# ComputationalPhysiology/oasisx

Hardware: AMD Instinct MI355X
Metric: time-steps/sec, 3D Taylor-Green 128^3 P2-P1 (with pressure-CG SpMV GB/s in roofline) (higher is better)
Workload: dtype f64

## Files before the change

### include/oasisx_hip.h

```cpp
#ifndef OASISX_HIP_H
#define OASISX_HIP_H

#include <stddef.h>
#include <stdint.h>

#ifdef __cplusplus
extern "C" {
#endif

#define OX_KV 2
#define OX_ROW_BLOCK_WAVES 8
#define OX_ROW_BLOCK_LDS (134 * 1024)
#define OX_SLICE 64

#define OX_CONVERGED_RTOL 2
#define OX_CONVERGED_ATOL 3
#define OX_CONVERGED_ITS 4
#define OX_DIVERGED_ITS (-3)
#define OX_DIVERGED_DTOL (-4)
#define OX_DIVERGED_BREAKDOWN (-5)
#define OX_DIVERGED_NANORINF (-9)

#define OX_KSP_CG 1
#define OX_KSP_BCGS 2
// ... 1 lines not shown
#define OX_KSP_BCGS_MERGED 4

#define OX_KSP_CG_MERGED 5

typedef struct {
  int64_t n_rows;
  int64_t n_cols;
  int32_t n_slices;
  int32_t n_dict;
  const int64_t *slice_ptr;
  const int32_t *cols;
  double *vals;
  const uint16_t *cols16;
  const int32_t *cbase;
  const uint8_t *vcode;
  const double *vdict;
  const int32_t *ib_slices;
  int32_t n_interior;
  int32_t n_wb_interior;
  const int64_t *ps_ptr;
  const uint32_t *ps_code;
  const int32_t *ps_base;
  const int32_t *wb_slices;
  const uint16_t *wb_waves;
  const int64_t *wb_ptr;
  const int32_t *wlist;
  const int64_t *wt_ptr;
  const uint16_t *wcode;
  const uint8_t *wvcode;
  int32_t n_wblocks;
  int32_t w_max;
  int32_t levels;
  int32_t w_cap;
} ox_sell;
#define OX_SPMV_LEVELS(mask) (32 | ((mask) & 31))

typedef struct {
  int32_t gdim;
  int32_t reserved;
  int64_t n_cells;
  const double *geom;
} ox_cells;

typedef struct {
  int32_t n_slices;
  int32_t nd;
  const int64_t *adj_ptr;
  const int32_t *adj_cell;
  const uint8_t *adj_loc;
} ox_adj;

typedef struct ox_dist ox_dist;

typedef struct {
  int32_t reason[4];
  int32_t its[4];
  double rnorm[4];
  double bnorm[4];
  int32_t resumed[4];
} ox_ksp_result;

typedef struct ox_mesh ox_mesh;
typedef struct ox_space ox_space;
typedef struct ox_rect ox_rect;

typedef struct {
  int32_t gdim, tile_bits;
  int64_t n_vertices, n_cells;
// ... 65 lines not shown
                       int on_device, const double *lo, const double *span, int lattice, int tile_bits,
                       int64_t n_cells_whole, ox_mesh **out);
int ox_space_create_part(const ox_mesh *mesh, int degree, int window, const int32_t *owner, int64_t n_initial, int rank,
                         int64_t n_dofs_whole, ox_space **out);
int ox_space_view(const ox_space *space, ox_space_info *view);
int ox_space_windows(ox_space *space, ox_window_info *view);
int ox_space_windows_split(ox_space *space, int split_entries, ox_window_info *view);
int ox_space_destroy(ox_space *space);
int ox_rect_create(const ox_space *rows, const ox_space *cols, ox_rect **out);
int ox_rect_view(const ox_rect *rect, ox_rect_info *view);
int ox_rect_destroy(ox_rect *rect);
int ox_value_dictionary(const double *vals, int64_t n_slots, int ncomp, void *codes, double *dict, int *n_dict,
                        void *stream);
int ox_pair_stream_size(const ox_sell *A, const int32_t *row_len, int64_t *ps_ptr, int64_t *n_codes, void *stream);
int ox_window_retile(const ox_sell *A, const int64_t *wt_ptr, const void *src, int elem_bytes, void *dst, void *stream);
int ox_pair_stream_fill(const ox_sell *A, const int32_t *row_len, int64_t *ps_ptr, uint32_t *ps_code,
                        int32_t *ps_base, int64_t *n_wide, void *stream);
int ox_malloc(size_t bytes, void **out);
int ox_free(void *p);
int ox_memset(void *p, int value, size_t bytes, void *stream);
int ox_synchronize(void *stream);

int ox_version(void);
const char *ox_last_error(void);
int ox_sell_kv(void);
int ox_device_info(int *n_cu, char *name, int name_len);

int ox_spmv(const ox_sell *A, const double *x, double *y, int ncomp, const ox_dist *dist,
            void *stream);

int ox_sell_compress_cols(const ox_sell *A, uint16_t *cols16, int32_t *cbase, int64_t *n_compressed,
                          void *stream);

int ox_spmv_multi(int v2s, int gdim, const ox_sell *A, const double *x, const double *base, double scale,
                  double *y, const ox_dist *dist, void *stream);
int ox_assemble_rect(int family, int row_degree, int col_degree, const ox_cells *cells, const ox_adj *adj,
                     const uint8_t *adj_pos, int pw, const ox_sell *A, void *stream);

int ox_axpby(int64_t n, double a, const double *x, double b, const double *y, double *z,
             void *stream);
int ox_dot(int64_t n_rows, int ncomp, const double *x, const double *y, double *out_host,
           const ox_dist *dist, void *stream);

int ox_set_bc(double *b, const int32_t *dofs, const double *g, int64_t n, int ncomp, int comp,
              void *stream);

int ox_scatter_add(double *b, const int32_t *rows, const double *y, int64_t n, int ncomp, int comp,
                   double scale, void *stream);

int ox_zero_rows(const ox_sell *A, const int32_t *rows, int64_t n, double diag, void *stream);
int ox_zero_rows_au(const ox_sell *A, const int32_t *rows, int64_t n, double diag, double *au,
                    const double *u1, int ncomp, void *stream);
int ox_zero_rows_cols(const ox_sell *A, const uint8_t *is_bc, double diag, void *stream);

int ox_assemble_matrix(int kind, int degree, const ox_cells *cells, const int32_t *cell_dofs,
                       const ox_adj *adj, const uint8_t *adj_pos, int pw, const ox_sell *A,
                       int n_bins, const int64_t *bin_ptr_host, const int32_t *bin_slices,
                       const int32_t *bin_width_host, void *stream);
int ox_assemble_weights(int degree, const ox_cells *cells, const ox_adj *adj, int64_t n_rows,
                        double *w, void *stream);
int ox_assemble_load_vector(const ox_cells *cells, const ox_adj *adj, int64_t n_rows, int n_d, int n_q,
                            const double *wphi, const double *fq, double *b, void *stream);

int ox_assemble_first(int degree, const ox_cells *cells, const int32_t *cell_dofs,
                      const ox_adj *adj, const uint8_t *adj_pos, int pw, const ox_sell *A,
                      const ox_sell *M, const ox_sell *K, const double *uab,
// ... 190 lines not shown
```

### oasisx_amd/_lib.py

```python
from __future__ import annotations

import ctypes as C
import os

_HERE = os.path.dirname(os.path.abspath(__file__))
LIB_PATH = os.environ.get("OX_LIB_PATH") or os.path.join(_HERE, "liboasisx_hip.so")

KSP_CG, KSP_BCGS, KSP_CG_SINGLE, KSP_BCGS_MERGED, KSP_CG_MERGED = 1, 2, 3, 4, 5
KSP_CG_MG = 6
MG_MAX_DEGREE = 8
ROW_BLOCK_WAVES, ROW_BLOCK_LDS = 8, 134 * 1024
CONVERGED_RTOL, CONVERGED_ATOL, CONVERGED_ITS = 2, 3, 4
DIVERGED_ITS, DIVERGED_DTOL, DIVERGED_BREAKDOWN, DIVERGED_NANORINF = -3, -4, -5, -9


class OasisxHipError(RuntimeError):
    pass


class ox_sell(C.Structure):
    _fields_ = [
        ("n_rows", C.c_int64),
        ("n_cols", C.c_int64),
        ("n_slices", C.c_int32),
        ("n_dict", C.c_int32),
        ("slice_ptr", C.c_void_p),
        ("cols", C.c_void_p),
        ("vals", C.c_void_p),
        ("cols16", C.c_void_p),
        ("cbase", C.c_void_p),
        ("vcode", C.c_void_p),
        ("vdict", C.c_void_p),
        ("ib_slices", C.c_void_p),
        ("n_interior", C.c_int32),
        ("n_wb_interior", C.c_int32),
        ("ps_ptr", C.c_void_p),
        ("ps_code", C.c_void_p),
        ("ps_base", C.c_void_p),
        ("wb_slices", C.c_void_p),
        ("wb_waves", C.c_void_p),
        ("wb_ptr", C.c_void_p),
        ("wlist", C.c_void_p),
        ("wt_ptr", C.c_void_p),
        ("wcode", C.c_void_p),
        ("wvcode", C.c_void_p),
        ("n_wblocks", C.c_int32),
        ("w_max", C.c_int32),
        ("levels", C.c_int32),
        ("w_cap", C.c_int32),
    ]


class ox_window_info(C.Structure):
    _fields_ = [
        ("n_wblocks", C.c_int32),
        ("w_max", C.c_int32),
        ("n_list", C.c_int64),
        ("n_tiles", C.c_int64),
        ("n_over_16bit", C.c_int64),
        ("wb_slices", C.c_void_p),
        ("wb_waves", C.c_void_p),
        ("wb_ptr", C.c_void_p),
        ("wlist", C.c_void_p),
        ("wt_ptr", C.c_void_p),
        ("wcode", C.c_void_p),
    ]


class ox_cells(C.Structure):
    _fields_ = [
        ("gdim", C.c_int32),
        ("reserved", C.c_int32),
        ("n_cells", C.c_int64),
        ("geom", C.c_void_p),
    ]


class ox_adj(C.Structure):
    _fields_ = [
        ("n_slices", C.c_int32),
        ("nd", C.c_int32),
        ("adj_ptr", C.c_void_p),
# ... 113 lines not shown
_P = C.c_void_p
_I = C.c_int
_L = C.c_int64
_D = C.c_double

SIGNATURES = {
    "ox_version": (_I, []),
    "ox_last_error": (C.c_char_p, []),
    "ox_sell_kv": (_I, []),
    "ox_device_info": (_I, [C.POINTER(_I), C.c_char_p, _I]),
    "ox_mesh_create": (_I, [_P, _L, _P, _L, _I, _I, _I, C.POINTER(_P)]),
    "ox_mesh_view": (_I, [_P, C.POINTER(ox_mesh_info)]),
    "ox_mesh_destroy": (_I, [_P]),
    "ox_space_create": (_I, [_P, _I, _I, C.POINTER(_P)]),
    "ox_space_create_ordered": (_I, [_P, _I, _I, _I, C.POINTER(_P)]),
    "ox_mesh_create_sub": (_I, [_P, _L, _P, _L, _I, _I, C.POINTER(_D), C.POINTER(_D), _I, _I, _L, C.POINTER(_P)]),
    "ox_space_create_part": (_I, [_P, _I, _I, _P, _L, _I, _L, C.POINTER(_P)]),
    "ox_space_view": (_I, [_P, C.POINTER(ox_space_info)]),
    "ox_space_windows": (_I, [_P, C.POINTER(ox_window_info)]),
    "ox_space_windows_split": (_I, [_P, _I, C.POINTER(ox_window_info)]),
    "ox_space_destroy": (_I, [_P]),
    "ox_rect_create": (_I, [_P, _P, C.POINTER(_P)]),
    "ox_rect_view": (_I, [_P, C.POINTER(ox_rect_info)]),
    "ox_rect_destroy": (_I, [_P]),
    "ox_value_dictionary": (_I, [_P, _L, _I, _P, _P, C.POINTER(_I), _P]),
    "ox_pair_stream_size": (_I, [C.POINTER(ox_sell), _P, _P, C.POINTER(_L), _P]),
    "ox_pair_stream_fill": (_I, [C.POINTER(ox_sell), _P, _P, _P, _P, C.POINTER(_L), _P]),
    "ox_malloc": (_I, [C.c_size_t, C.POINTER(_P)]),
    "ox_free": (_I, [_P]),
    "ox_memset": (_I, [_P, _I, C.c_size_t, _P]),
    "ox_synchronize": (_I, [_P]),
    "ox_spmv": (_I, [C.POINTER(ox_sell), _P, _P, _I, _P, _P]),
    "ox_sell_compress_cols": (_I, [C.POINTER(ox_sell), _P, _P, C.POINTER(_L), _P]),
    "ox_spmv_multi": (_I, [_I, _I, C.POINTER(ox_sell), _P, _P, _D, _P, _P, _P]),
    "ox_assemble_rect": (_I, [_I, _I, _I, C.POINTER(ox_cells), C.POINTER(ox_adj), _P, _I, C.POINTER(ox_sell), _P]),
    "ox_axpby": (_I, [_L, _D, _P, _D, _P, _P, _P]),
    "ox_dot": (_I, [_L, _I, _P, _P, C.POINTER(_D), _P, _P]),
    "ox_set_bc": (_I, [_P, _P, _P, _L, _I, _I, _P]),
    "ox_scatter_add": (_I, [_P, _P, _P, _L, _I, _I, _D, _P]),
    "ox_zero_rows": (_I, [C.POINTER(ox_sell), _P, _L, _D, _P]),
    "ox_zero_rows_au": (_I, [C.POINTER(ox_sell), _P, _L, _D, _P, _P, _I, _P]),
    "ox_zero_rows_cols": (_I, [C.POINTER(ox_sell), _P, _D, _P]),
    "ox_assemble_matrix": (_I, [_I, _I, C.POINTER(ox_cells), _P, C.POINTER(ox_adj), _P, _I,
                                C.POINTER(ox_sell), _I, C.POINTER(_L), _P, C.POINTER(C.c_int32), _P]),
    "ox_assemble_weights": (_I, [_I, C.POINTER(ox_cells), C.POINTER(ox_adj), _L, _P, _P]),
    "ox_assemble_load_vector": (_I, [C.POINTER(ox_cells), C.POINTER(ox_adj), _L, _I, _I, _P, _P, _P, _P]),
    "ox_assemble_first": (_I, [_I, C.POINTER(ox_cells), _P, C.POINTER(ox_adj), _P, _I,
                               C.POINTER(ox_sell), C.POINTER(ox_sell), C.POINTER(ox_sell), _P, _P, _P, _P, _D,
                               _D, _I, C.POINTER(_L), _P, C.POINTER(C.c_int32), _P]),
    "ox_assemble_first_au": (_I, [_I, C.POINTER(ox_cells), _P, C.POINTER(ox_adj), _P, _I,
                                  C.POINTER(ox_sell), C.POINTER(ox_sell), C.POINTER(ox_sell), _P, _P, _P, _P, _D,
                                  _D, _I, C.POINTER(_L), _P, C.POINTER(C.c_int32), _P, _P]),
    "ox_assemble_matrix_blocks": (_I, [_I, _I, C.POINTER(ox_cells), _P, C.POINTER(ox_adj), _P, _I, C.POINTER(ox_sell), _I, _P,
                                       _L, _P]),
    "ox_assemble_first_blocks": (_I, [_I, C.POINTER(ox_cells), _P, C.POINTER(ox_adj), _P, _I,
                                      C.POINTER(ox_sell), C.POINTER(ox_sell), C.POINTER(ox_sell), _P, _P, _P, _P, _D,
                                      _D, _I, _P, _L, _P, _P]),
    "ox_eddy_viscosity": (_I, [_I, _I, C.POINTER(ox_cells), _P, _P, _D, _P, _P]),
    "ox_assemble_first_au_nut": (_I, [_I, C.POINTER(ox_cells), _P, C.POINTER(ox_adj), _P, _I,
                                      C.POINTER(ox_sell), C.POINTER(ox_sell), C.POINTER(ox_sell), _P, _P, _P, _P, _D,
                                      _D, _I, C.POINTER(_L), _P, C.POINTER(C.c_int32), _P, _P, _P]),
    "ox_assemble_first_blocks_nut": (_I, [_I, C.POINTER(ox_cells), _P, C.POINTER(ox_adj), _P, _I,
                                          C.POINTER(ox_sell), C.POINTER(ox_sell), C.POINTER(ox_sell), _P, _P, _P, _P, _D,
                                          _D, _I, _P, _L, _P, _P, _P]),
    "ox_viscosity_law": (_I, [_I, _I, C.POINTER(ox_cells), _P, _P, C.POINTER(_D), _I, _P, _P]),
    "ox_assemble_stress_transpose": (_I, [_I, C.POINTER(ox_cells), _P, C.POINTER(ox_adj), _L, _P, _P, _D, _P, _P]),
# ... 117 lines not shown
```

### oasisx_amd/csrc/ox_spmv.hip

```cpp
#include "ox_common.h"
#include "ox_kernels.h"
#include <stdlib.h>
#include <type_traits>

thread_local char ox_err_buf[512] = "";

extern "C" int ox_version(void) { return 100; }
extern "C" const char *ox_last_error(void) { return ox_err_buf; }
extern "C" int ox_sell_kv(void) { return OX_KV; }

extern "C" int ox_device_info(int *n_cu, char *name, int name_len) {
  int dev = 0;
  OX_HIP(hipGetDevice(&dev));
  hipDeviceProp_t p;
  OX_HIP(hipGetDeviceProperties(&p, dev));
  if (n_cu) *n_cu = p.multiProcessorCount;
  if (name && name_len > 0) {
    strncpy(name, p.gcnArchName, name_len - 1);
    name[name_len - 1] = 0;
  }
  return 0;
}

template <int NC, int EPI, int VAR>
// ... 34 lines not shown
    const int64_t base = A.slice_ptr[slice];
    const int npair = (int)((A.slice_ptr[slice + 1] - base) >> 7);
    const double2 *__restrict__ vp = reinterpret_cast<const double2 *>(A.vals + base) + lane;
    typedef double v2d __attribute__((ext_vector_type(2)));
    typedef int v2i __attribute__((ext_vector_type(2)));
    typedef unsigned short v2h __attribute__((ext_vector_type(2)));
    const unsigned short *__restrict__ vcp =
        (VAR & 4) ? reinterpret_cast<const unsigned short *>(A.vcode + base) + lane : nullptr;
    auto load_vals = [&](int k) {
      double2 v;
      if (VAR & 4) {
        const unsigned cc = __builtin_nontemporal_load(vcp + (size_t)k * 64);
        v.x = dict[cc & 0xff];
        v.y = dict[cc >> 8];
      } else if (VAR & 1) {
        const v2d vv = __builtin_nontemporal_load(reinterpret_cast<const v2d *>(vp + (size_t)k * 64));
        v.x = vv.x;
        v.y = vv.y;
      } else {
        v = vp[(size_t)k * 64];
      }
      return v;
    };
    auto mac = [&](double2 v, int c0, int c1) {
      const double *x0 = x + (size_t)c0 * NC;
      const double *x1 = x + (size_t)c1 * NC;
#pragma unroll
      for (int cc = 0; cc < NC; ++cc) acc[cc] = fma(v.x, x0[cc], acc[cc]);
#pragma unroll
      for (int cc = 0; cc < NC; ++cc) acc[cc] = fma(v.y, x1[cc], acc[cc]);
    };
    const int2 *__restrict__ cb =
        (VAR & 2) ? reinterpret_cast<const int2 *>(A.cbase) + (base >> 7) : nullptr;
    if ((VAR & 2) && cb[0].x >= 0) {
      const v2h *__restrict__ hp = reinterpret_cast<const v2h *>(A.cols16 + base) + lane;
#pragma unroll 4
      for (int k = 0; k < npair; ++k) {
        const double2 v = load_vals(k);
        const v2h d = __builtin_nontemporal_load(hp + (size_t)k * 64);
        const int2 b = cb[k];
        const int dx = d.x, dy = d.y;
        mac(v, ((dx & 0x8000) ? b.y : b.x) + (dx & 0x7fff), ((dy & 0x8000) ? b.y : b.x) + (dy & 0x7fff));
      }
    } else {
      const int2 *__restrict__ cp = reinterpret_cast<const int2 *>(A.cols + base) + lane;
#pragma unroll 4
      for (int k = 0; k < npair; ++k) {
        const double2 v = load_vals(k);
        int2 c;
        if (VAR & 1) {
          const v2i ci = __builtin_nontemporal_load(reinterpret_cast<const v2i *>(cp + (size_t)k * 64));
          c.x = ci.x;
          c.y = ci.y;
        } else {
          c = cp[(size_t)k * 64];
        }
        mac(v, c.x, c.y);
      }
    }
    if (row < A.n_rows) {
      if (EPI == OX_EPI_BCGS_V || EPI == OX_EPI_BCGS_T || EPI == OX_EPI_BCGS_T5) {
        const double d = dinv[row];
#pragma unroll
        for (int c = 0; c < NC; ++c) acc[c] *= d;
      }
#pragma unroll
      for (int c = 0; c < NC; ++c) y[row * NC + c] = acc[c];
// ... 373 lines not shown
            const double dd = ED.code ? ED.dict[ED.code[row]] : dinv[row];
            s[c] = fma(x[row * NC + c], acc[c], s[c]);
            s[NC + c] = fma(acc[c], dd * acc[c], s[NC + c]);
          }
        }
      }
    }
  }
  if (EPI != OX_EPI_NONE) {
    ox_block_sum_256<NV>(s, red);
    if (threadIdx.x == 0) {
#pragma unroll
      for (int i = 0; i < NV; ++i) partial[(size_t)blockIdx.x * NV + i] = s[i];
    }
  }
}

#include <mutex>
static const int *ox_zero_flag(hipStream_t st) {
  static std::mutex mu;
  static int *z[16] = {};
  int dev = 0;
  if (hipGetDevice(&dev) != hipSuccess || dev < 0 || dev >= 16) return nullptr;
  std::lock_guard<std::mutex> lock(mu);
  if (!z[dev]) {
    int *p = nullptr;
    if (hipMalloc(&p, 64) != hipSuccess) return nullptr;
    if (hipMemsetAsync(p, 0, 64, st) != hipSuccess || hipStreamSynchronize(st) != hipSuccess) return nullptr;
    z[dev] = p;
  }
  return z[dev];
}

#define OX_SPMV_DEFAULT_VARIANT 31
static inline int spmv_levels(const ox_sell *A) { return (A->levels & 32) ? (A->levels & 31) : OX_SPMV_DEFAULT_VARIANT; }

static int spmv_window_cap(const ox_sell *A, int ncomp, const int32_t *list) {
  if (list && !(A->ib_slices && (list == A->ib_slices || list == A->ib_slices + A->n_interior))) return 0;
  if (!(spmv_levels(A) & 16) || !A->wcode || !A->wt_ptr || !A->wlist || !A->wb_ptr || !A->wb_slices ||
      !A->wb_waves || A->n_wblocks <= 0 || ncomp < 1 || ncomp > 3)
    return 0;
  const int dflt = ncomp == 1 ? 6144 : (ncomp == 2 ? 3072 : 2176);
  const int cap = A->w_cap > 0 ? A->w_cap : dflt;
  return A->w_max < cap ? A->w_max : cap;
}
static inline int spmv_window_grid_n(int nblocks) { return (nblocks + 7) & ~7; }
static inline void spmv_window_range(const ox_sell *A, const int32_t *list, int n_list, int *first, int *count) {
  if (!list) *first = 0, *count = A->n_wblocks;
  else if (list == A->ib_slices && n_list == A->n_interior) *first = 0, *count = A->n_wb_interior;
  else *first = A->n_wb_interior, *count = A->n_wblocks - A->n_wb_interior;
}

static thread_local OxEpiDinv g_epi_dinv{nullptr, nullptr};
void ox_spmv_set_epilogue_dinv(const uint8_t *code, const double *dict) { g_epi_dinv = OxEpiDinv{code, dict}; }

static int spmv_launch_list(const ox_sell *A, const double *x, double *y, int ncomp, int epi,
                            const double *dinv, const double *aux, double *partial, const int *done,
                            hipStream_t st, const int32_t *list, int n_list) {
  const int nblk = list ? ox_spmv_blocks_n(n_list) : ox_spmv_blocks(A);
  if (nblk == 0) return 0;
  const int lv = spmv_levels(A);
  int var = (A->cols16 && A->cbase) ? (lv & 7) : (lv & 1);
  const bool pairs = (lv & 8) && A->ps_ptr && A->ps_code && A->ps_base;
  if ((var & 6) != 6 || !A->vcode || !A->vdict || A->n_dict < 1 || A->n_dict > 256) var &= 3;
  else var = 7;
  const int w_cap = pairs ? 0 : spmv_window_cap(A, ncomp, list);
  if (w_cap > 0) {
    const bool codes = var == 7 && A->wvcode;
    int wb0 = 0, wbn = 0;
    spmv_window_range(A, list, n_list, &wb0, &wbn);
    if (wbn == 0) return 0;
    const int wgrid = spmv_window_grid_n(wbn);
    const size_t lds = (size_t)w_cap * ncomp * sizeof(double);
#define OX_WIN_CASE(NC, E)                                                                                          \
  if (ncomp == NC && epi == E) {                                                                                    \
    auto go = [&](auto kern) -> int {                                                                               \
      if (lds > 48 * 1024)                                                                                          \
        OX_HIP(hipFuncSetAttribute(reinterpret_cast<const void *>(kern), hipFuncAttributeMaxDynamicSharedMemorySize, \
                                   (int)lds));                                                                      \
      if (ox_prof_on) ox_prof_start(OX_TAG_SPMV(NC, E), st, A->n_rows);                                             \
      hipLaunchKernelGGL(kern, dim3(wgrid), dim3(256), lds, st, *A, x, y, dinv, aux, partial, done, w_cap, g_epi_dinv, wb0, wbn); \
      if (ox_prof_on) ox_prof_stop(st);                                                                             \
      OX_LAUNCH_CHECK();                                                                                            \
      return 0;                                                                                                     \
    };                                                                                                              \
    return codes ? go(k_spmv_win<NC, E, 5>) : go(k_spmv_win<NC, E, 1>);                                             \
  }
#define OX_WIN_NC(NC)                                                                                   \
  OX_WIN_CASE(NC, OX_EPI_NONE) OX_WIN_CASE(NC, OX_EPI_DOT) OX_WIN_CASE(NC, OX_EPI_BCGS_V) OX_WIN_CASE(NC, OX_EPI_BCGS_T) \
  OX_WIN_CASE(NC, OX_EPI_BCGS_T5) OX_WIN_CASE(NC, OX_EPI_CG_M2)
    OX_WIN_NC(1) OX_WIN_NC(2) OX_WIN_NC(3)
#undef OX_WIN_NC
#undef OX_WIN_CASE
  }
#define OX_SPMV_LAUNCH(NC, E, V)                                                                   \
  hipLaunchKernelGGL((k_spmv<NC, E, V>), dim3(nblk), dim3(256), 0, st, *A, x, y, dinv, aux, partial, done, list, n_list, g_epi_dinv)
#define OX_SPMV_CASE(NC, E)                                                                     \
  if (ncomp == NC && epi == E) {                                                                \
    if (ox_prof_on) ox_prof_start(OX_TAG_SPMV(NC, E), st, A->n_rows);                                      \
    if (var == 7 && pairs) {                                                                    \
      const int *dz = done ? done : ox_zero_flag(st);                                             \
      if (!dz) OX_FAIL("ox_spmv: no device flag");                                              \
      hipLaunchKernelGGL((k_spmv_ps<NC, E>), dim3(nblk), dim3(256), 0, st, *A, x, y, dinv, aux, partial, dz, list, n_list, g_epi_dinv); \
    } else if (var == 7) OX_SPMV_LAUNCH(NC, E, 7);                                              \
    else if (var == 3) OX_SPMV_LAUNCH(NC, E, 3);                                                \
    else if (var == 2) OX_SPMV_LAUNCH(NC, E, 2);                                                \
    else if (var == 1) OX_SPMV_LAUNCH(NC, E, 1);                                                \
    else OX_SPMV_LAUNCH(NC, E, 0);                                                              \
    if (ox_prof_on) ox_prof_stop(st);                                                           \
    OX_LAUNCH_CHECK();                                                                          \
    return 0;                                                                                   \
  }
#define OX_SPMV_NC(NC)               \
  OX_SPMV_CASE(NC, OX_EPI_NONE)      \
  OX_SPMV_CASE(NC, OX_EPI_DOT)       \
  OX_SPMV_CASE(NC, OX_EPI_BCGS_V)    \
  OX_SPMV_CASE(NC, OX_EPI_BCGS_T)    \
  OX_SPMV_CASE(NC, OX_EPI_BCGS_T5)   \
  OX_SPMV_CASE(NC, OX_EPI_CG_M2)
  OX_SPMV_NC(1) OX_SPMV_NC(2) OX_SPMV_NC(3)
#undef OX_SPMV_NC
#undef OX_SPMV_CASE
  OX_FAIL("ox_spmv: unsupported ncomp=%d epi=%d", ncomp, epi);
}

int ox_spmv_launch(const ox_sell *A, const double *x, double *y, int ncomp, int epi,
                   const double *dinv, const double *aux, double *partial, const int *done,
                   hipStream_t st) {
  return spmv_launch_list(A, x, y, ncomp, epi, dinv, aux, partial, done, st, nullptr, 0);
}

static bool ox_overlap_on(const ox_sell *A, const ox_dist *dist) {
  if (!(dist && dist->n_peers > 0 && A->ib_slices && A->n_interior > 0)) return false;
  if (dist->overlap >= 0) return dist->overlap != 0;
  return !(dist->comm && !dist->p2p && !dist->halo_cb);
}

// ... 74 lines not shown
    d.y = !fits ? 0 : (unsigned short)(fy ? (0x8000 | (c.y - lo2)) : (c.y - lo));
    hp[(size_t)k * 64] = d;
    if (lane == 0) bp[k] = make_int2(lo, lo2 == BIG ? lo : lo2);
  }
  if (lane == 0 && npair > 0) {
    if (!ok) bp[0].x = -1;
    else if (n_ok) atomicAdd(n_ok, (unsigned long long)npair * 128ull);
  }
}

extern "C" int ox_sell_compress_cols(const ox_sell *A, uint16_t *cols16, int32_t *cbase,
                                     int64_t *n_compressed, void *stream) {
  if (!A || !cols16 || !cbase) OX_FAIL("ox_sell_compress_cols: null argument");
  hipStream_t st = ox_stream(stream);
  if (n_compressed) *n_compressed = 0;
  if (A->n_slices == 0) return 0;
  unsigned long long *cnt = nullptr;
  if (n_compressed) {
    OX_HIP(hipMalloc(&cnt, sizeof(*cnt)));
    OX_HIP(hipMemsetAsync(cnt, 0, sizeof(*cnt), st));
  }
  hipLaunchKernelGGL(k_compress_cols, dim3((A->n_slices + 3) / 4), dim3(256), 0, st, *A, cols16, cbase, cnt);
  OX_LAUNCH_CHECK();
  if (n_compressed) {
    unsigned long long h = 0;
    OX_HIP(hipMemcpyAsync(&h, cnt, sizeof(h), hipMemcpyDeviceToHost, st));
    OX_HIP(hipStreamSynchronize(st));
    OX_HIP(hipFree(cnt));
    *n_compressed = (int64_t)h;
  }
  return 0;
}

template <int GD, int V2S, bool DICT>
__global__ __launch_bounds__(256) void k_spmv_multi(ox_sell A, const double *__restrict__ x,
                                                    const double *__restrict__ base, double scale,
                                                    double *__restrict__ y) {
  __shared__ double dict[DICT ? 256 : 1];
  if constexpr (DICT) {
    if ((int)threadIdx.x < A.n_dict) dict[threadIdx.x] = A.vdict[threadIdx.x];
    __syncthreads();
  }
  const int ngroups = (A.n_slices + 3) >> 2;
  const int chunk = (ngroups + 7) >> 3;
  const int g = (blockIdx.x & 7) * chunk + (blockIdx.x >> 3);
  if ((int)(blockIdx.x >> 3) >= chunk || g >= ngroups) return;
  const int slice = __builtin_amdgcn_readfirstlane(g * 4 + (threadIdx.x >> 6)), lane = threadIdx.x & 63;
  if (slice >= A.n_slices) return;
  const int64_t row = (int64_t)slice * 64 + lane;
  const int64_t sbase = A.slice_ptr[slice];
  const int npair = (int)((A.slice_ptr[slice + 1] - sbase) >> 7);
  const int2 *__restrict__ cp = reinterpret_cast<const int2 *>(A.cols + sbase) + lane;
  double acc[GD];
#pragma unroll
  for (int d = 0; d < GD; ++d) acc[d] = 0.0;
  auto mac = [&](const double (&v)[2 * GD], int c0, int c1) {
    if (V2S) {
      const double *x0 = x + (size_t)c0 * GD, *x1 = x + (size_t)c1 * GD;
#pragma unroll
      for (int d = 0; d < GD; ++d) acc[0] = fma(v[GD + d], x1[d], fma(v[d], x0[d], acc[0]));
    } else {
      const double x0 = x[c0], x1 = x[c1];
#pragma unroll
      for (int d = 0; d < GD; ++d) acc[d] = fma(v[GD + d], x1, fma(v[d], x0, acc[d]));
    }
  };
// ... 503 lines not shown
```

### oasisx_amd/fem.py

```python
from __future__ import annotations

import ctypes as C
import itertools

import numpy as np
import torch

from . import _lib
from .mesh import Mesh

KV = 2
SLICE = 64
default_scalar_type = np.float64


def local_edges(gdim: int):
    return [(1, 2), (0, 2), (0, 1)] if gdim == 2 else [(2, 3), (1, 3), (1, 2), (0, 3), (0, 2), (0, 1)]


import os as _os


def default_tile_bits(mesh: Mesh) -> int:
    env = _os.environ.get("OX_TILE_BITS")
# ... 118 lines not shown

def row_blocks(widths: np.ndarray):
    cap = _lib.ROW_BLOCK_LDS // 8
    blk, used, cnt, big = [0], 0, 0, 0
    for s_, w in enumerate(np.asarray(widths, dtype=np.int64)):
        e = int(w) * SLICE
        if e > cap:
            return np.zeros(1, dtype=np.int32), 0
        if cnt == _lib.ROW_BLOCK_WAVES or used + e > cap:
            blk.append(s_)
            used, cnt = 0, 0
        used, cnt = used + e, cnt + 1
        big = max(big, used)
    if len(widths):
        blk.append(len(widths))
    return np.asarray(blk, dtype=np.int32), int(big)


class SellPattern:

    def __init__(self, n_rows, n_cols, slice_ptr, cols, row_len, widths, nnz=None, row_blk=None):
        self.n_rows, self.n_cols = int(n_rows), int(n_cols)
        self.slice_ptr = slice_ptr
        self.cols = cols
        self.row_len = row_len
        self.widths = widths
        self.n_slices = int(widths.shape[0])
        self.size = int(cols.shape[0])
        self.nnz = int(row_len.sum().item()) if nnz is None else int(nnz)
        self.device = cols.device
        self.dist = None
        self.cols16 = self.cbase = None
        self.frac16 = 0.0
        self.ib_slices, self.n_interior = None, 0
        w = torch.from_numpy(widths.astype(np.int64))
        order = torch.argsort(w, stable=True)
        ws = w[order]
        uw, counts = torch.unique_consecutive(ws, return_counts=True)
        self.bin_width, self.bin_ptr = merge_small_bins(uw.numpy().astype(np.int32),
                                                        np.concatenate([[0], np.cumsum(counts.numpy())]).astype(np.int64))
        self.bin_slices = order.to(torch.int32).to(self.device)
        if row_blk is None:
            bp, big = row_blocks(widths)
            row_blk = (torch.from_numpy(bp).to(self.device), big)
        self.row_blk_ptr, self.row_blk_entries = row_blk
        self.n_row_blocks = int(self.row_blk_ptr.shape[0]) - 1

    def blocks_args(self):
        return self.n_row_blocks, _lib.ptr(self.row_blk_ptr), int(self.row_blk_entries)

    def split_interior(self, n_owned: int):
        if self.n_slices == 0 or self.size == 0:
            return
        width = torch.from_numpy(self.widths.astype(np.int64)).to(self.device) * SLICE
        sl = torch.repeat_interleave(torch.arange(self.n_slices, device=self.device), width)
        ghost = torch.zeros(self.n_slices, dtype=torch.int32, device=self.device)
        ghost.index_put_((sl,), (self.cols >= n_owned).to(torch.int32), accumulate=True)
        interior = torch.nonzero(ghost == 0).reshape(-1)
        boundary = torch.nonzero(ghost > 0).reshape(-1)
        self.ib_slices = torch.cat([interior, boundary]).to(torch.int32).contiguous()
        self.n_interior = int(interior.shape[0])
        self._slice_has_ghost = ghost > 0
        self.order_window_blocks()

    def order_window_blocks(self):
        if getattr(self, "wcode", None) is None or getattr(self, "_slice_has_ghost", None) is None \
# ... 77 lines not shown
        del uk_all
        ub = torch.div(ukey, ncols, rounding_mode="floor")
        wb_ptr[1:] = torch.cumsum(torch.bincount(ub, minlength=nb), 0)
        wlist = (ukey - ub * ncols).to(torch.int32)
        w_all = wb_ptr[1:] - wb_ptr[:-1]
        w_max = int(w_all.max().item())
        big = w_all > 65535
        for s0 in range(0, ns, chunk_slices):
            s1 = min(ns, s0 + chunk_slices)
            a, b = int(sp[s0].item()), int(sp[s1].item())
            bs = torch.repeat_interleave(blk_of_slice[s0:s1], slot_per_slice[s0:s1])
            code = torch.searchsorted(ukey, bs * ncols + self.cols[a:b].to(torch.int64)) - wb_ptr[bs]
            code = torch.where(big[bs], torch.zeros_like(code), code)
            wcode[a:b] = (code & 0xffff).to(torch.int32).to(torch.int16)
        npair = width // KV
        wt_ptr = torch.zeros(ns + 1, dtype=torch.int64, device=dev)
        wt_ptr[1:] = torch.cumsum((npair + 1) // 2, 0)
        n_tiles = int(wt_ptr[-1].item())
        plain = _lib.ox_sell(self.n_rows, self.n_cols, self.n_slices, 0, self.slice_ptr.data_ptr(), self.cols.data_ptr())
        tiled = torch.empty(n_tiles * 256, dtype=torch.int16, device=dev)
        _lib.check(_lib.load().ox_window_retile(C.byref(plain), _lib.ptr(wt_ptr), _lib.ptr(wcode), 2, _lib.ptr(tiled),
                                                _lib.current_stream()), "ox_window_retile")
        del wcode
        self.wb_slices, self.wb_waves = wb_slices.contiguous(), sched.to(torch.int32).to(torch.int16).contiguous()
        self.wb_ptr, self.wlist, self.wcode, self.wt_ptr = wb_ptr, wlist.contiguous(), tiled, wt_ptr
        self.n_wblocks, self.w_max = nb, w_max
        wq = torch.quantile(w_all.to(torch.float64), torch.tensor([0.5, 0.9, 0.99], dtype=torch.float64, device=dev))
        self.w_stats = {"blocks": nb, "w_mean": float(w_all.to(torch.float64).mean().item()), "w_max": w_max,
                        "w_p50_p90_p99": [int(v) for v in wq.tolist()],
                        "share_over_2176": float((w_all > 2176).to(torch.float64).mean().item()),
                        "list_bytes": int(wlist.numel()) * 4, "over_16bit": int(big.sum().item())}
        return True

    def struct(self, vals: torch.Tensor, compress: bool = True) -> _lib.ox_sell:
        assert vals.shape[0] % self.size == 0 and vals.dtype == torch.float64
        c16 = cb = None
        if compress and self.device.type == "cuda" and self.size > 0:
            if self.cols16 is None:
                self.cols16 = torch.empty(self.size, dtype=torch.int16, device=self.device)
                self.cbase = torch.empty(2 * (self.size // (SLICE * KV)), dtype=torch.int32, device=self.device)
                plain = _lib.ox_sell(self.n_rows, self.n_cols, self.n_slices, 0, self.slice_ptr.data_ptr(),
                                     self.cols.data_ptr(), None, None, None, None, None)
                n16 = C.c_int64(0)
                _lib.check(_lib.load().ox_sell_compress_cols(C.byref(plain), _lib.ptr(self.cols16),
                                                             _lib.ptr(self.cbase), C.byref(n16),
                                                             _lib.current_stream()), "ox_sell_compress_cols")
                self.frac16 = n16.value / self.size
            c16, cb = self.cols16.data_ptr(), self.cbase.data_ptr()
        S = _lib.ox_sell(self.n_rows, self.n_cols, self.n_slices, 0, self.slice_ptr.data_ptr(),
                         self.cols.data_ptr(), vals.data_ptr(), c16, cb, None, None)
        if self.ib_slices is not None:
            S.ib_slices, S.n_interior = self.ib_slices.data_ptr(), self.n_interior
        if getattr(self, "wcode", None) is not None:
            S.wb_slices, S.wb_waves, S.wb_ptr = self.wb_slices.data_ptr(), self.wb_waves.data_ptr(), self.wb_ptr.data_ptr()
            S.wlist, S.wcode, S.n_wblocks, S.w_max = self.wlist.data_ptr(), self.wcode.data_ptr(), self.n_wblocks, self.w_max
            S.wt_ptr = self.wt_ptr.data_ptr()
            S.n_wb_interior = int(getattr(self, "n_wb_interior", None) or 0)
        return S

    def bins_args(self):
        return (int(self.bin_width.shape[0]), self.bin_ptr.ctypes.data_as(C.POINTER(C.c_int64)),
                _lib.ptr(self.bin_slices), self.bin_width.ctypes.data_as(C.POINTER(C.c_int32)))

    def slot_rows_k(self):
        sp = self.slice_ptr.cpu().numpy()
        o = np.arange(self.size, dtype=np.int64)
        s = np.searchsorted(sp, o, side="right") - 1
        loc = o - sp[s]
        k = (loc // (SLICE * KV)) * KV + loc % KV
        lane = (loc % (SLICE * KV)) // KV
        return s * SLICE + lane, k

    def to_csr(self, vals: torch.Tensor):
        import scipy.sparse as sp

        rows, k = self.slot_rows_k()
        rl = np.zeros(self.n_slices * SLICE, dtype=np.int64)
        rl[: self.n_rows] = self.row_len.cpu().numpy()
        ok = k < rl[rows]
        A = sp.coo_matrix((vals.cpu().numpy()[ok], (rows[ok], self.cols.cpu().numpy()[ok])),
                          shape=(self.n_rows, self.n_cols)).tocsr()
        A.sort_indices()
        return A

    def values_from_csr(self, A) -> torch.Tensor:
# ... 1132 lines not shown
```

### oasisx_amd/la.py

```python
from __future__ import annotations

import ctypes as C
import os

import torch

from . import _lib
from .fem import SellPattern


def _env_int(name):
    try:
        return int(os.environ[name])
    except (KeyError, ValueError):
        return None


ENV_SPMV_LEVELS = _env_int("OX_SPMV_VARIANT")
ENV_WIN_CAP = _env_int("OX_WIN_CAP")


def _apply_schedule(struct, levels, w_cap):
    struct.levels = 0 if levels is None else (32 | (int(levels) & 31))
    struct.w_cap = 0 if not w_cap else int(w_cap)


class SellMatrix:

    def __init__(self, pattern: SellPattern, symmetric: bool = False, name: str = "A"):
        self.pattern = pattern
        self.vals = pattern.new_values()
        self.symmetric = symmetric
        self.name = name
        self.version = 0
        self.vcode = self.vdict = self._vc_version = None
        self.ps_ptr = self.ps_code = self.ps_base = None
        self.ps_wide = 0
        self.wvcode = None
        self._struct = pattern.struct(self.vals)
        self.levels, self.w_cap = ENV_SPMV_LEVELS, ENV_WIN_CAP
        _apply_schedule(self._struct, self.levels, self.w_cap)

    def set_levels(self, mask: int | None, w_cap: int | None = None):
        self.levels = mask
        if w_cap is not None:
            self.w_cap = w_cap or None
        _apply_schedule(self._struct, self.levels, self.w_cap)

    @property
    def struct(self) -> _lib.ox_sell:
        return self._struct

    def ref(self):
        if self._vc_version is not None and self._vc_version != self.version:
            self._drop_codes()
        return C.byref(self._struct)

    def _drop_codes(self):
        self.vcode = self.vdict = self._vc_version = None
        self._struct.vcode = self._struct.vdict = None
        self._struct.n_dict = 0
        self.ps_ptr = self.ps_code = self.ps_base = None
        self._struct.ps_ptr = self._struct.ps_code = self._struct.ps_base = None
        self.wvcode = None
        self._struct.wvcode = None

    def freeze(self, block: int = 1 << 27, pairs: str = "auto") -> bool:
        P = self.pattern
        if P.device.type != "cuda" or P.cols16 is None or P.size == 0:
            return False
        code = torch.empty(P.size, dtype=torch.uint8, device=P.device)
        vdict = torch.zeros(256, dtype=torch.float64, device=P.device)
        nd = C.c_int(0)
        _lib.check(_lib.load().ox_value_dictionary(_lib.ptr(self.vals), P.size, 1, _lib.ptr(code), _lib.ptr(vdict),
                                                   C.byref(nd), _lib.current_stream()), "ox_value_dictionary")
        if nd.value == 0:
            return False
        self.vcode, self.vdict = code, vdict[: nd.value]
        self._vc_version = self.version
        self._struct.vcode, self._struct.vdict = self.vcode.data_ptr(), self.vdict.data_ptr()
        self._struct.n_dict = int(nd.value)
        if pairs != "never":
            self._build_pair_stream(force=pairs == "always")
        if getattr(P, "wt_ptr", None) is not None and self.ps_code is None:
            self.wvcode = torch.empty(int(P.wt_ptr[-1].item()) * 256, dtype=torch.uint8, device=P.device)
            _lib.check(_lib.load().ox_window_retile(C.byref(self._struct), _lib.ptr(P.wt_ptr), _lib.ptr(self.vcode), 1,
                                                    _lib.ptr(self.wvcode), _lib.current_stream()), "ox_window_retile")
            self._struct.wvcode = self.wvcode.data_ptr()
        return True

    def _build_pair_stream(self, force: bool = False):
        P, lib = self.pattern, _lib.load()
        ps_ptr = torch.empty(P.n_slices + 1, dtype=torch.int64, device=P.device)
        n = C.c_int64(0)
        _lib.check(lib.ox_pair_stream_size(C.byref(self._struct), _lib.ptr(P.row_len), _lib.ptr(ps_ptr), C.byref(n),
                                           _lib.current_stream()), "ox_pair_stream_size")
        if n.value == 0 or (not force and n.value > 0.72 * P.size):
            return
        code = torch.empty(n.value, dtype=torch.int32, device=P.device)
        base = torch.empty(2 * (n.value // 256), dtype=torch.int32, device=P.device)
        wide = C.c_int64(0)
        _lib.check(lib.ox_pair_stream_fill(C.byref(self._struct), _lib.ptr(P.row_len), _lib.ptr(ps_ptr), _lib.ptr(code),
                                           _lib.ptr(base), C.byref(wide), _lib.current_stream()), "ox_pair_stream_fill")
        self.ps_ptr, self.ps_code, self.ps_base, self.ps_wide = ps_ptr, code, base, int(wide.value)
        self._struct.ps_ptr, self._struct.ps_code, self._struct.ps_base = ps_ptr.data_ptr(), code.data_ptr(), base.data_ptr()

    def getSize(self):
        return (self.pattern.n_rows, self.pattern.n_cols)

    def to_scipy(self):
        return self.pattern.to_csr(self.vals)

    def mult(self, x: torch.Tensor, y: torch.Tensor, ncomp: int = 1):
        lib = _lib.load()
        _lib.check(lib.ox_spmv(self.ref(), _lib.ptr(x), _lib.ptr(y), ncomp, self.pattern.dist,
                               _lib.current_stream()), "ox_spmv")
# ... 60 lines not shown
```

Measured before the change: 12.19.

## Add uniform-slice SpMV path storing one column base and value code per slice column

Detects SELL slices where each column of the slice has lane-affine column indices (col = base + lane), and optionally identical value codes across lanes. For those slices it stores one base per column and one dictionary code per column, so the SpMV kernel reads a per-slice int2 base and packed codes instead of per-lane cols16/vcode arrays. This cuts index and code traffic on structured-mesh matrices. In exchange it adds census and build kernels at setup, extra struct fields, and new kernel variants enabled by default through the widened levels mask.

```diff
diff --git a/include/oasisx_hip.h b/include/oasisx_hip.h
--- a/include/oasisx_hip.h
+++ b/include/oasisx_hip.h
@@ -57,8 +57,12 @@
   int32_t w_max;
   int32_t levels;
   int32_t w_cap;
+  const int32_t *us_off;
+  const int32_t *us_base;
+  const int32_t *us_coff;
+  const uint8_t *us_code;
 } ox_sell;
-#define OX_SPMV_LEVELS(mask) (32 | ((mask) & 31))
+#define OX_SPMV_LEVELS(mask) (64 | ((mask) & 63))
 
 typedef struct {
   int32_t gdim;
@@ -190,6 +194,11 @@
 int ox_sell_compress_cols(const ox_sell *A, uint16_t *cols16, int32_t *cbase, int64_t *n_compressed,
                           void *stream);
 
+int ox_uniform_census(const ox_sell *A, int32_t *flag, int host, void *stream);
+int ox_uniform_bases(const ox_sell *A, const int32_t *us_off, int32_t *us_base, int host, void *stream);
+int ox_uniform_codes(const ox_sell *A, const int32_t *us_off, int32_t *us_coff, uint8_t *us_code, int host,
+                     void *stream);
+
 int ox_spmv_multi(int v2s, int gdim, const ox_sell *A, const double *x, const double *base, double scale,
                   double *y, const ox_dist *dist, void *stream);
 int ox_assemble_rect(int family, int row_degree, int col_degree, const ox_cells *cells, const ox_adj *adj,
diff --git a/oasisx_amd/_lib.py b/oasisx_amd/_lib.py
--- a/oasisx_amd/_lib.py
+++ b/oasisx_amd/_lib.py
@@ -48,6 +48,10 @@
         ("w_max", C.c_int32),
         ("levels", C.c_int32),
         ("w_cap", C.c_int32),
+        ("us_off", C.c_void_p),
+        ("us_base", C.c_void_p),
+        ("us_coff", C.c_void_p),
+        ("us_code", C.c_void_p),
     ]
 
 
@@ -227,6 +231,9 @@
     "ox_synchronize": (_I, [_P]),
     "ox_spmv": (_I, [C.POINTER(ox_sell), _P, _P, _I, _P, _P]),
     "ox_sell_compress_cols": (_I, [C.POINTER(ox_sell), _P, _P, C.POINTER(_L), _P]),
+    "ox_uniform_census": (_I, [C.POINTER(ox_sell), _P, _I, _P]),
+    "ox_uniform_bases": (_I, [C.POINTER(ox_sell), _P, _P, _I, _P]),
+    "ox_uniform_codes": (_I, [C.POINTER(ox_sell), _P, _P, _P, _I, _P]),
     "ox_spmv_multi": (_I, [_I, _I, C.POINTER(ox_sell), _P, _P, _D, _P, _P, _P]),
     "ox_assemble_rect": (_I, [_I, _I, _I, C.POINTER(ox_cells), C.POINTER(ox_adj), _P, _I, C.POINTER(ox_sell), _P]),
     "ox_axpby": (_I, [_L, _D, _P, _D, _P, _P, _P]),
diff --git a/oasisx_amd/csrc/ox_spmv.hip b/oasisx_amd/csrc/ox_spmv.hip
--- a/oasisx_amd/csrc/ox_spmv.hip
+++ b/oasisx_amd/csrc/ox_spmv.hip
@@ -90,7 +90,29 @@
     };
     const int2 *__restrict__ cb =
         (VAR & 2) ? reinterpret_cast<const int2 *>(A.cbase) + (base >> 7) : nullptr;
-    if ((VAR & 2) && cb[0].x >= 0) {
+    const int uo = (VAR & 8) ? A.us_off[slice] : -1;
+    const int uco = ((VAR & 12) == 12) ? A.us_coff[slice] : -1;
+    if ((VAR & 12) == 12 && uco >= 0) {
+      const int2 *__restrict__ ub = reinterpret_cast<const int2 *>(A.us_base + uco);
+      const unsigned *__restrict__ uc = reinterpret_cast<const unsigned *>(A.us_code + uco);
+#pragma unroll 4
+      for (int k = 0; k < npair; ++k) {
+        const int2 b = ub[k];
+        const unsigned cc = uc[k >> 1] >> ((k & 1) * 16);
+        double2 v;
+        v.x = dict[cc & 0xff];
+        v.y = dict[(cc >> 8) & 0xff];
+        mac(v, b.x + lane, b.y + lane);
+      }
+    } else if ((VAR & 8) && uo >= 0) {
+      const int2 *__restrict__ ub = reinterpret_cast<const int2 *>(A.us_base + uo);
+#pragma unroll 4
+      for (int k = 0; k < npair; ++k) {
+        const double2 v = load_vals(k);
+        const int2 b = ub[k];
+        mac(v, b.x + lane, b.y + lane);
+      }
+    } else if ((VAR & 2) && cb[0].x >= 0) {
       const v2h *__restrict__ hp = reinterpret_cast<const v2h *>(A.cols16 + base) + lane;
 #pragma unroll 4
       for (int k = 0; k < npair; ++k) {
@@ -530,8 +552,8 @@
   return z[dev];
 }
 
-#define OX_SPMV_DEFAULT_VARIANT 31
-static inline int spmv_levels(const ox_sell *A) { return (A->levels & 32) ? (A->levels & 31) : OX_SPMV_DEFAULT_VARIANT; }
+#define OX_SPMV_DEFAULT_VARIANT 63
+static inline int spmv_levels(const ox_sell *A) { return (A->levels & 64) ? (A->levels & 63) : OX_SPMV_DEFAULT_VARIANT; }
 
 static int spmv_window_cap(const ox_sell *A, int ncomp, const int32_t *list) {
   if (list && !(A->ib_slices && (list == A->ib_slices || list == A->ib_slices + A->n_interior))) return 0;
@@ -563,6 +585,7 @@
   if ((var & 6) != 6 || !A->vcode || !A->vdict || A->n_dict < 1 || A->n_dict > 256) var &= 3;
   else var = 7;
   const int w_cap = pairs ? 0 : spmv_window_cap(A, ncomp, list);
+  const bool uni = (lv & 32) && A->us_off && A->us_base && (var != 7 || (A->us_coff && A->us_code));
   if (w_cap > 0) {
     const bool codes = var == 7 && A->wvcode;
     int wb0 = 0, wbn = 0;
@@ -600,7 +623,9 @@
       const int *dz = done ? done : ox_zero_flag(st);                                             \
       if (!dz) OX_FAIL("ox_spmv: no device flag");                                              \
       hipLaunchKernelGGL((k_spmv_ps<NC, E>), dim3(nblk), dim3(256), 0, st, *A, x, y, dinv, aux, partial, dz, list, n_list, g_epi_dinv); \
-    } else if (var == 7) OX_SPMV_LAUNCH(NC, E, 7);                                              \
+    } else if (var == 7 && uni) OX_SPMV_LAUNCH(NC, E, 15);                                      \
+    else if (var == 7) OX_SPMV_LAUNCH(NC, E, 7);                                                \
+    else if (var == 3 && uni) OX_SPMV_LAUNCH(NC, E, 11);                                        \
     else if (var == 3) OX_SPMV_LAUNCH(NC, E, 3);                                                \
     else if (var == 2) OX_SPMV_LAUNCH(NC, E, 2);                                                \
     else if (var == 1) OX_SPMV_LAUNCH(NC, E, 1);                                                \
@@ -741,6 +766,116 @@
   return 0;
 }
 
+template <typename T>
+__host__ __device__ inline bool ox_us_lane_ok(const T *a, int64_t base, int width, int lane, int shift) {
+  bool ok = true;
+  for (int k = 0; k < width; ++k) {
+    const int64_t e = base + (int64_t)(k >> 1) * 128 + (k & 1);
+    ok = ok && ((int)a[e + 2 * lane] - shift * lane == (int)a[e]);
+  }
+  return ok;
+}
+static inline int ox_us_width(const ox_sell &A, int slice) { return (int)((A.slice_ptr[slice + 1] - A.slice_ptr[slice]) >> 6); }
+
+__global__ __launch_bounds__(256) void k_uniform_census(ox_sell A, int32_t *__restrict__ flag) {
+  const int slice = blockIdx.x * 4 + (threadIdx.x >> 6), lane = threadIdx.x & 63;
+  if (slice >= A.n_slices) return;
+  const int64_t base = A.slice_ptr[slice];
+  const int width = (int)((A.slice_ptr[slice + 1] - base) >> 6);
+  const int ok = ox_wave_min_all(ox_us_lane_ok(A.cols, base, width, lane, 1) ? 1 : 0);
+  if (lane == 0) flag[slice] = (width > 0 && ok) ? 1 : 0;
+}
+
+__global__ __launch_bounds__(256) void k_uniform_bases(ox_sell A, const int32_t *__restrict__ us_off,
+                                                       int32_t *__restrict__ us_base) {
+  const int slice = blockIdx.x * 4 + (threadIdx.x >> 6), lane = threadIdx.x & 63;
+  if (slice >= A.n_slices) return;
+  const int off = us_off[slice];
+  if (off < 0) return;
+  const int64_t base = A.slice_ptr[slice];
+  const int width = (int)((A.slice_ptr[slice + 1] - base) >> 6);
+  for (int k = lane; k < ((width + 3) & ~3); k += 64)
+    us_base[(int64_t)off + k] = k < width ? A.cols[base + (int64_t)(k >> 1) * 128 + (k & 1)] : 0;
+}
+
+__global__ __launch_bounds__(256) void k_uniform_codes(ox_sell A, const int32_t *__restrict__ us_off,
+                                                       int32_t *__restrict__ us_coff, uint8_t *__restrict__ us_code) {
+  const int slice = blockIdx.x * 4 + (threadIdx.x >> 6), lane = threadIdx.x & 63;
+  if (slice >= A.n_slices) return;
+  const int off = us_off[slice];
+  if (off < 0) {
+    if (lane == 0) us_coff[slice] = -1;
+    return;
+  }
+  const int64_t base = A.slice_ptr[slice];
+  const int width = (int)((A.slice_ptr[slice + 1] - base) >> 6);
+  const int ok = ox_wave_min_all(ox_us_lane_ok(A.vcode, base, width, lane, 0) ? 1 : 0);
+  if (lane == 0) us_coff[slice] = ok ? off : -1;
+  for (int k = lane; k < ((width + 3) & ~3); k += 64)
+    us_code[(int64_t)off + k] = (ok && k < width) ? A.vcode[base + (int64_t)(k >> 1) * 128 + (k & 1)] : (uint8_t)0;
+}
+
+extern "C" int ox_uniform_census(const ox_sell *A, int32_t *flag, int host, void *stream) {
+  if (!A || !flag || (A->n_slices > 0 && (!A->slice_ptr || !A->cols))) OX_FAIL("ox_uniform_census: null argument");
+  if (A->n_slices == 0) return 0;
+  if (host) {
+    for (int s = 0; s < A->n_slices; ++s) {
+      const int width = ox_us_width(*A, s);
+      bool ok = width > 0;
+      for (int lane = 0; lane < 64 && ok; ++lane) ok = ox_us_lane_ok(A->cols, A->slice_ptr[s], width, lane, 1);
+      flag[s] = ok ? 1 : 0;
+    }
+    return 0;
+  }
+  hipLaunchKernelGGL(k_uniform_census, dim3((A->n_slices + 3) / 4), dim3(256), 0, ox_stream(stream), *A, flag);
+  OX_LAUNCH_CHECK();
+  return 0;
+}
+
+extern "C" int ox_uniform_bases(const ox_sell *A, const int32_t *us_off, int32_t *us_base, int host, void *stream) {
+  if (!A || !us_off || (A->n_slices > 0 && (!A->slice_ptr || !A->cols))) OX_FAIL("ox_uniform_bases: null argument");
+  if (A->n_slices == 0) return 0;
+  if (host) {
+    for (int s = 0; s < A->n_slices; ++s) {
+      if (us_off[s] < 0) continue;
+      if (!us_base) OX_FAIL("ox_uniform_bases: null argument");
+      const int width = ox_us_width(*A, s);
+      for (int k = 0; k < ((width + 3) & ~3); ++k)
+        us_base[(int64_t)us_off[s] + k] = k < width ? A->cols[A->slice_ptr[s] + (int64_t)(k >> 1) * 128 + (k & 1)] : 0;
+    }
+    return 0;
+  }
+  hipLaunchKernelGGL(k_uniform_bases, dim3((A->n_slices + 3) / 4), dim3(256), 0, ox_stream(stream), *A, us_off, us_base);
+  OX_LAUNCH_CHECK();
+  return 0;
+}
+
+extern "C" int ox_uniform_codes(const ox_sell *A, const int32_t *us_off, int32_t *us_coff, uint8_t *us_code, int host,
+                                void *stream) {
+  if (!A || !us_off || !us_coff || (A->n_slices > 0 && (!A->slice_ptr || !A->vcode)))
+    OX_FAIL("ox_uniform_codes: null argument");
+  if (A->n_slices == 0) return 0;
+  if (host) {
+    for (int s = 0; s < A->n_slices; ++s) {
+      us_coff[s] = -1;
+      if (us_off[s] < 0) continue;
+      if (!us_code) OX_FAIL("ox_uniform_codes: null argument");
+      const int width = ox_us_width(*A, s);
+      bool ok = true;
+      for (int lane = 0; lane < 64 && ok; ++lane) ok = ox_us_lane_ok(A->vcode, A->slice_ptr[s], width, lane, 0);
+      if (ok) us_coff[s] = us_off[s];
+      for (int k = 0; k < ((width + 3) & ~3); ++k)
+        us_code[(int64_t)us_off[s] + k] =
+            (ok && k < width) ? A->vcode[A->slice_ptr[s] + (int64_t)(k >> 1) * 128 + (k & 1)] : (uint8_t)0;
+    }
+    return 0;
+  }
+  hipLaunchKernelGGL(k_uniform_codes, dim3((A->n_slices + 3) / 4), dim3(256), 0, ox_stream(stream), *A, us_off, us_coff,
+                     us_code);
+  OX_LAUNCH_CHECK();
+  return 0;
+}
+
 template <int GD, int V2S, bool DICT>
 __global__ __launch_bounds__(256) void k_spmv_multi(ox_sell A, const double *__restrict__ x,
                                                     const double *__restrict__ base, double scale,
diff --git a/oasisx_amd/fem.py b/oasisx_amd/fem.py
--- a/oasisx_amd/fem.py
+++ b/oasisx_amd/fem.py
@@ -174,6 +174,9 @@
         self.dist = None
         self.cols16 = self.cbase = None
         self.frac16 = 0.0
+        self.us_off = self.us_base = None
+        self.n_uniform = self.n_upos = 0
+        self._us_done = False
         self.ib_slices, self.n_interior = None, 0
         w = torch.from_numpy(widths.astype(np.int64))
         order = torch.argsort(w, stable=True)
@@ -317,6 +320,36 @@
                         "list_bytes": int(wlist.numel()) * 4, "over_16bit": int(big.sum().item())}
         return True
 
+    def uniform_census(self, host: bool = False):
+        lib, st = _lib.load(), _lib.current_stream()
+        self._us_done = True
+        self.us_off = self.us_base = None
+        self.n_uniform = self.n_upos = 0
+        if self.n_slices == 0 or self.size == 0:
+            return None, None
+        plain = _lib.ox_sell(self.n_rows, self.n_cols, self.n_slices, 0, self.slice_ptr.data_ptr(), self.cols.data_ptr())
+        flag = torch.zeros(self.n_slices, dtype=torch.int32, device=self.device)
+        _lib.check(lib.ox_uniform_census(C.byref(plain), _lib.ptr(flag), int(host), st), "ox_uniform_census")
+        n_uni = int(flag.sum().item())
+        if n_uni == 0:
+            return None, None
+        w4 = (torch.from_numpy(self.widths.astype(np.int64)).to(self.device) + 3) // 4 * 4 * flag.to(torch.int64)
+        end = torch.cumsum(w4, 0)
+        n_pos = int(end[-1].item())
+        assert n_pos < 2 ** 31
+        us_off = torch.where(flag > 0, end - w4, torch.full_like(end, -1)).to(torch.int32).contiguous()
+        us_base = torch.zeros(n_pos, dtype=torch.int32, device=self.device)
+        _lib.check(lib.ox_uniform_bases(C.byref(plain), _lib.ptr(us_off), _lib.ptr(us_base), int(host), st),
+                   "ox_uniform_bases")
+        self.us_off, self.us_base, self.n_uniform, self.n_upos = us_off, us_base, n_uni, n_pos
+        return us_off, us_base
+
+    def uniform_shares(self):
+        if self.us_off is None:
+            return 0.0, 0.0
+        w = torch.from_numpy(self.widths.astype(np.int64)).to(self.device)
+        return self.n_uniform / self.n_slices, float((w * (self.us_off >= 0)).sum().item()) * SLICE / self.size
+
     def struct(self, vals: torch.Tensor, compress: bool = True) -> _lib.ox_sell:
         assert vals.shape[0] % self.size == 0 and vals.dtype == torch.float64
         c16 = cb = None
@@ -332,10 +365,14 @@
                                                              _lib.current_stream()), "ox_sell_compress_cols")
                 self.frac16 = n16.value / self.size
             c16, cb = self.cols16.data_ptr(), self.cbase.data_ptr()
+            if not self._us_done:
+                self.uniform_census()
         S = _lib.ox_sell(self.n_rows, self.n_cols, self.n_slices, 0, self.slice_ptr.data_ptr(),
                          self.cols.data_ptr(), vals.data_ptr(), c16, cb, None, None)
         if self.ib_slices is not None:
             S.ib_slices, S.n_interior = self.ib_slices.data_ptr(), self.n_interior
+        if compress and self.us_off is not None:
+            S.us_off, S.us_base = self.us_off.data_ptr(), self.us_base.data_ptr()
         if getattr(self, "wcode", None) is not None:
             S.wb_slices, S.wb_waves, S.wb_ptr = self.wb_slices.data_ptr(), self.wb_waves.data_ptr(), self.wb_ptr.data_ptr()
             S.wlist, S.wcode, S.n_wblocks, S.w_max = self.wlist.data_ptr(), self.wcode.data_ptr(), self.n_wblocks, self.w_max
diff --git a/oasisx_amd/la.py b/oasisx_amd/la.py
--- a/oasisx_amd/la.py
+++ b/oasisx_amd/la.py
@@ -21,7 +21,7 @@
 
 
 def _apply_schedule(struct, levels, w_cap):
-    struct.levels = 0 if levels is None else (32 | (int(levels) & 31))
+    struct.levels = 0 if levels is None else (64 | (int(levels) & 63))
     struct.w_cap = 0 if not w_cap else int(w_cap)
 
 
@@ -37,6 +37,8 @@
         self.ps_ptr = self.ps_code = self.ps_base = None
         self.ps_wide = 0
         self.wvcode = None
+        self.us_coff = self.us_code = None
+        self.n_code_uniform = 0
         self._struct = pattern.struct(self.vals)
         self.levels, self.w_cap = ENV_SPMV_LEVELS, ENV_WIN_CAP
         _apply_schedule(self._struct, self.levels, self.w_cap)
@@ -64,6 +66,9 @@
         self._struct.ps_ptr = self._struct.ps_code = self._struct.ps_base = None
         self.wvcode = None
         self._struct.wvcode = None
+        self.us_coff = self.us_code = None
+        self._struct.us_coff = self._struct.us_code = None
+        self.n_code_uniform = 0
 
     def freeze(self, block: int = 1 << 27, pairs: str = "auto") -> bool:
         P = self.pattern
@@ -82,6 +87,13 @@
         self._struct.n_dict = int(nd.value)
         if pairs != "never":
             self._build_pair_stream(force=pairs == "always")
+        if P.us_off is not None:
+            self.us_coff = torch.empty(P.n_slices, dtype=torch.int32, device=P.device)
+            self.us_code = torch.empty(P.n_upos, dtype=torch.uint8, device=P.device)
+            _lib.check(_lib.load().ox_uniform_codes(C.byref(self._struct), _lib.ptr(P.us_off), _lib.ptr(self.us_coff),
+                                                    _lib.ptr(self.us_code), 0, _lib.current_stream()), "ox_uniform_codes")
+            self.n_code_uniform = int((self.us_coff >= 0).sum().item())
+            self._struct.us_coff, self._struct.us_code = self.us_coff.data_ptr(), self.us_code.data_ptr()
         if getattr(P, "wt_ptr", None) is not None and self.ps_code is None:
             self.wvcode = torch.empty(int(P.wt_ptr[-1].item()) * 256, dtype=torch.uint8, device=P.device)
             _lib.check(_lib.load().ox_window_retile(C.byref(self._struct), _lib.ptr(P.wt_ptr), _lib.ptr(self.vcode), 1,
```

Result: faster. 12.38, median of 6 (+1.5%).
